# facebookresearch/DRTK

Hardware: AMD Instinct MI355X
Metric: Mpixels/sec fwd+bwd, 100k-tri @ 2048x2048, 1/2/4/8 GPU; HBM BW % (higher is better)
Workload: dtype f32; 1 GPU; 8 views/GPU x 1 GPU, 100k-tri UV-sphere head mesh (F=100352, V=50400), 2048x2048, C=16 attribute channels, transform+rasterize+render+interpolate+mask+edge_grad_estimator+loss fwd+bwd; views_per_gpu=8, triangles=100352, vertices=50400, height=2048, width=2048, channels=16, grad_reset=set_to_none, parallelism=single GPU

## Files before the change

drtk_amd/csrc/common.hpp:

```cpp
#pragma once

#include <hip/hip_runtime.h>

#include <atomic>
#include <stdint.h>
#include <string>
#include <type_traits>

#include "drtk_amd.h"

namespace drtk_amd {

constexpr int kWave = 64;
constexpr int kBlock = 256;

template <typename T>
struct Eps;
template <>
struct Eps<float> {
  static __host__ __device__ constexpr float value() { return 1e-8f; }
};
template <>
struct Eps<double> {
  static __host__ __device__ constexpr double value() { return 1e-16; }
// ... 17 lines not shown
template <typename T>
__device__ __forceinline__ T min3(T a, T b, T c) {
  T m = a;
  if (b < m) m = b;
  if (c < m) m = c;
  return m;
}
template <typename T>
__device__ __forceinline__ T max3(T a, T b, T c) {
  T m = a;
  if (m < b) m = b;
  if (m < c) m = c;
  return m;
}

__device__ __forceinline__ int lane_id() {
  return __builtin_amdgcn_mbcnt_hi(~0u, __builtin_amdgcn_mbcnt_lo(~0u, 0u));
}

template <typename T>
__device__ __forceinline__ void atomic_add_global(T* p, T v) {
  unsafeAtomicAdd(p, v);
}

template <typename T>
using NtQuad = T __attribute__((ext_vector_type(4)));
template <typename T>
__device__ __forceinline__ NtQuad<T> nt_load4(const T* p) {
  return __builtin_nontemporal_load(reinterpret_cast<const NtQuad<T>*>(p));
}
template <typename T>
__device__ __forceinline__ void nt_store4(T* p, T a, T b, T c, T d) {
  __builtin_nontemporal_store(NtQuad<T>{a, b, c, d}, reinterpret_cast<NtQuad<T>*>(p));
}

__device__ __forceinline__ int xcd_tile(int b, int n, int strip) {
  constexpr int kXcds = 8;
  const int group = kXcds * strip;
  const int base = b / group * group;
  const int r = b - base;
  const int left = n - base;
  if (left >= group) return base + (r % kXcds) * strip + r / kXcds;
  const int s = left / kXcds;
  if (r < s * kXcds) return base + (r % kXcds) * s + r / kXcds;
  return b;
}
__device__ __forceinline__ int tile_index(int strip) {
  const int b = static_cast<int>(blockIdx.x);
  return strip <= 1 ? b : xcd_tile(b, static_cast<int>(gridDim.x), strip);
}

#ifdef DRTK_AMD_ABLATION
int debug_flags();
#define DRTK_DBG(mask, bit) (((mask) & (bit)) != 0)
#else
constexpr int debug_flags() { return 0; }
#define DRTK_DBG(mask, bit) false
#endif
inline int xcd_strip(int64_t tiles_per_16_rows) {
  const int forced = (debug_flags() >> 10) & 1023;
  if (forced) return forced;
  return tiles_per_16_rows < 2 ? 2 : static_cast<int>(tiles_per_16_rows);
}

int num_compute_units();

// ... 93 lines not shown
```

drtk_amd/csrc/edge_grad.hip:

```cpp
#include <cstdlib>

#include "common.hpp"
#include "segscatter.hpp"

namespace drtk_amd {
namespace {

template <typename T>
struct Vec4;
template <>
struct Vec4<float> {
  using type = float4;
};
template <>
struct Vec4<double> {
  using type = double4;
};

template <typename T>
using Quad = T __attribute__((ext_vector_type(4), aligned(sizeof(T))));

using BufferRsrc = __amdgpu_buffer_rsrc_t;
__device__ __forceinline__ BufferRsrc buffer_rsrc(const void* base, uint32_t bytes) {
  return __builtin_amdgcn_make_buffer_rsrc(const_cast<void*>(base), 0, static_cast<int>(bytes), 0x00020000);
}
__device__ __forceinline__ float as_float(uint32_t bits) {
  return __builtin_bit_cast(float, bits);
}
__device__ __forceinline__ int32_t buffer_load_i32(BufferRsrc r, uint32_t byte_offset) {
  return static_cast<int32_t>(__builtin_amdgcn_raw_buffer_load_b32(r, byte_offset, 0, 0));
}

__device__ __forceinline__ int prefix4(int cnt, unsigned long long lt, int& total) {
  const unsigned long long b0 = __ballot(cnt & 1), b1 = __ballot(cnt & 2), b2 = __ballot(cnt & 4);
  total = __popcll(b0) + 2 * __popcll(b1) + 4 * __popcll(b2);
  return __popcll(b0 & lt) + 2 * __popcll(b1 & lt) + 4 * __popcll(b2 & lt);
}

template <typename E, typename EntryOf>
__device__ __forceinline__ void append_flagged(uint32_t f, unsigned long long lt, int& n_all, E* list, EntryOf entry) {
  int t;
  int pos = n_all + prefix4(__popc(f), lt, t);
  n_all += t;
#pragma unroll
  for (int j = 0; j < 4; ++j) {
    if (f & (1u << j)) list[pos++] = entry(j);
  }
}

template <typename T>
struct TriInfo {
  T p0x, p0y, p1x, p1y;
  T v01x, v01y, v02x, v02y, v12x, v12y;
  T den;
  T nx, ny, nz;
  int32_t i0, i1, i2;
};

template <typename T>
__device__ __forceinline__ void tri_setup(TriInfo<T>& t, T p0x, T p0y, T p1x, T p1y, T p2x, T p2y) {
  t.p0x = p0x;
  t.p0y = p0y;
  t.p1x = p1x;
  t.p1y = p1y;
// ... 1090 lines not shown
```

drtk_amd/csrc/interpolate.hip:

```cpp
#include <string>

#include "common.hpp"
#include "segscatter.hpp"

namespace drtk_amd {
namespace {

template <typename T>
struct Vec4;
template <>
struct Vec4<float> {
  using type = float4;
};
template <>
struct Vec4<double> {
  using type = double4;
};

template <typename T, int VEC, int CV, bool PREFETCH = false, bool ANYW = false>
__global__ __launch_bounds__(kBlock) void interpolate_kernel(
    const T* __restrict__ attrs, const int32_t* __restrict__ vi,
    const int32_t* __restrict__ index_img, const T* __restrict__ bary_img, int64_t V, int C,
    int64_t vi_sN, int H, int W, T* __restrict__ out, int zero_background, int strip) {
  using V4 = typename Vec4<T>::type;
// ... 416 lines not shown
      }
    }
    if (ps + 1 < kPasses) load_face(tr_next, vn);
    if constexpr (HAS_VERT) {
      int dist;
      bool tail;
      run_rows16(tr, dist, tail);
      if (__ballot(covered) != 0) {
        T p[3 * CN];
#pragma unroll
        for (int k = 0; k < 3; ++k) {
#pragma unroll
          for (int c = 0; c < CN; ++c) p[k * CN + c] = g[c] * B[k];
        }
        run_sums_rows16<T, 3 * CN>(p, dist);
        if (tail && covered) table_add<T, 3, CN, kSlots>(t_keys[wave], t_vals[wave], kStride, cur, p, attr_grad_n, CN);
      }
    }
  }
  if constexpr (HAS_VERT) {
    wave_lds_sync();
    table_flush<T, TableAcc, kSlots>(t_keys[wave], t_vals[wave], kStride, CN, attr_grad_n, CN, 0);
  }
}

constexpr int kWideWaves = 4;
constexpr int kWideWavesF64 = 3;
constexpr int kPlaneLoadAux = 2;
constexpr int kAttrGroupsAhead = 1;
constexpr bool kAnycSplitLastGroup = true;
template <typename T, bool HAS_BARY, bool TABLE, int CH, bool ANYC>
__global__ __launch_bounds__(kBlock, (sizeof(T) == 8 ? kWideWavesF64 : kWideWaves)) void interpolate_backward_wide_kernel(
    const T* __restrict__ grad_out, const T* __restrict__ attrs, const int32_t* __restrict__ vi,
    const int32_t* __restrict__ index_img, const T* __restrict__ bary_img, int64_t V, int C,
    int64_t vi_sN, int H, int W, int tiles_x, T* __restrict__ attr_grad, T* __restrict__ bary_grad,
    int dbg, int strip, int log2_slots, int CG) {
  using V4 = typename Vec4<T>::type;
  static_assert(CH % 4 == 0 && CH >= 8 && CH <= 16, "chunks of 8 or 16 channels");
  constexpr int kWaves = kBlock / kWave;
  constexpr int kPasses = kTileRows / kWaves;
  static_assert(kPasses == 4, "row pipeline below is written for 4 rows per wave");
  __shared__ __attribute__((aligned(16))) T s_g[kWaves][CH * kRunPad];
  __shared__ __attribute__((aligned(16))) T s_b[kWaves][3 * kRunPad];
  __shared__ int32_t s_vid[kWaves][3 * kRunPad];
  __shared__ int32_t s_slot[TABLE ? kWaves : 1][TABLE ? 3 * kRunPad : 1];
  extern __shared__ __attribute__((aligned(16))) unsigned char s_table_raw[];
  TableAcc* const t_vals = reinterpret_cast<TableAcc*>(s_table_raw);
  int32_t* const t_keys = reinterpret_cast<int32_t*>(t_vals + (TABLE ? (size_t(C) << log2_slots) : 0));

  const int64_t HW = int64_t(H) * W;
  const int n = blockIdx.y;
  const int tile = tile_index(strip);
  const int tyi = tile / tiles_x, txi = tile - tyi * tiles_x;
  const int wave = threadIdx.x / kWave;
  const int lane = threadIdx.x & (kWave - 1);
  const int x = txi * kWave + lane;
  const int y0 = tyi * kTileRows + wave * kPasses;
  const T* attrs_n = attrs + int64_t(n) * V * C;
  const int32_t* vi_n = vi + int64_t(n) * vi_sN;
  T* attr_grad_n = attr_grad + int64_t(n) * V * CG;
  const T* go_n = grad_out + int64_t(n) * C * HW;
  const T* bary_n = bary_img + int64_t(n) * 3 * HW;
  T* bgrad_n = HAS_BARY ? bary_grad + int64_t(n) * 3 * HW : nullptr;
  if constexpr (TABLE) {
    for (int i = threadIdx.x; i < (C << log2_slots); i += kBlock) t_vals[i] = 0;
    for (int i = threadIdx.x; i < (1 << log2_slots); i += kBlock) t_keys[i] = -1;
  }

  auto load_tr = [&](int ps) -> int32_t {
    const int y = y0 + ps;
    return (ps < kPasses && x < W && y < H) ? index_img[int64_t(n) * HW + int64_t(y) * W + x] : -1;
  };
  auto load_face = [&](int32_t t, int32_t& a0, int32_t& a1, int32_t& a2) {
    a0 = a1 = a2 = 0;
    if (t != -1) {
      const int32_t* face = vi_n + int64_t(t) * 3;
      a0 = face[0], a1 = face[1], a2 = face[2];
    }
  };

  bool wave_fg;
  {
    int32_t t4[kPasses];
#pragma unroll
    for (int ps = 0; ps < kPasses; ++ps) t4[ps] = load_tr(ps);
    const bool any_fg = (t4[0] & t4[1] & t4[2] & t4[3]) != -1;
    wave_fg = __ballot(any_fg) != 0;
    bool tile_fg = wave_fg;
    if constexpr (TABLE) tile_fg = __syncthreads_or(wave_fg) != 0;
    if (!wave_fg) {
      if constexpr (HAS_BARY) {
        int yz = y0;
        asm volatile("" : "+v"(yz));
#pragma unroll
        for (int ps = 0; ps < kPasses; ++ps) {
          const int y = yz + ps;
          if (x < W && y < H) {
            T* bgp = bgrad_n + int64_t(y) * W + x;
            bgp[0] = T(0), bgp[HW] = T(0), bgp[2 * HW] = T(0);
          }
        }
      }
      if (!TABLE || !tile_fg) return;
    }
  }

  if (wave_fg) {
  T G[CH], B[3];
  const uint32_t plane_bytes = static_cast<uint32_t>(HW * int64_t(sizeof(T)));
  auto plane_load = [&](const T* plane, uint32_t byte_offset, bool exists) -> T {
    const __amdgpu_buffer_rsrc_t r = __builtin_amdgcn_make_buffer_rsrc(const_cast<T*>(plane), 0, exists ? static_cast<int>(plane_bytes) : 0, 0x00020000);
    if constexpr (sizeof(T) == 4) {
      return __builtin_bit_cast(T, __builtin_amdgcn_raw_buffer_load_b32(r, byte_offset, 0, kPlaneLoadAux));
    } else {
      return __builtin_bit_cast(T, __builtin_amdgcn_raw_buffer_load_b64(r, byte_offset, 0, kPlaneLoadAux));
    }
  };
  auto row_offset = [&](int ps) -> uint32_t {
    return (x < W && y0 + ps < H) ? static_cast<uint32_t>((y0 + ps) * W + x) * static_cast<uint32_t>(sizeof(T)) : plane_bytes;
  };
  auto load_row = [&](int ps, int c0, int cc, bool row_any, bool with_bary) {
    if (!row_any) return;
    const uint32_t bo = row_offset(ps);
    const T* plane = go_n + int64_t(c0) * HW;
#pragma unroll
    for (int q = 0; q < CH / 4; ++q) {
      if (4 * q < cc) {
#pragma unroll
        for (int c = 4 * q; c < 4 * q + 4; ++c) {
          G[c] = plane_load(plane, bo, !ANYC || c < cc);
          plane += HW;
        }
      }
    }
    if (with_bary) {
      const T* bplane = bary_n;
#pragma unroll
      for (int k = 0; k < 3; ++k) {
        B[k] = plane_load(bplane, bo, true);
        bplane += HW;
      }
    }
  };
  int32_t tr = load_tr(0), tr_n = load_tr(1), tr_nn = -1;
  int32_t v0, v1, v2, vn0 = 0, vn1 = 0, vn2 = 0;
  load_face(tr, v0, v1, v2);
#pragma unroll
  for (int c = 0; c < CH; ++c) G[c] = T(0);
  B[0] = B[1] = B[2] = T(0);
  load_row(0, 0, min(CH, C), __ballot(tr != -1) != 0, true);
  unsigned long long heads = 0, cov = 0;
  T bg0 = T(0), bg1 = T(0), bg2 = T(0);
  int ps = 0, c0 = 0;
#pragma unroll 1
  for (;;) {
    const bool covered = tr != -1;
    if (c0 == 0) {
      if (ps + 1 < kPasses) {
        load_face(tr_n, vn0, vn1, vn2);
        tr_nn = load_tr(ps + 2);
      }
#pragma unroll
      for (int k = 0; k < 3; ++k) s_b[wave][k * kRunPad + lane] = B[k];
      s_vid[wave][0 * kRunPad + lane] = v0;
      s_vid[wave][1 * kRunPad + lane] = v1;
      s_vid[wave][2 * kRunPad + lane] = v2;
      run_masks(tr, heads, cov);
      bg0 = bg1 = bg2 = T(0);
      if constexpr (TABLE) {
        int s0 = -1, s1 = -1, s2 = -1;
        if (covered && ((heads >> lane) & 1ull) && !DRTK_DBG(dbg, 2)) {
          s0 = table_slot_rt(t_keys, v0, log2_slots);
          s1 = table_slot_rt(t_keys, v1, log2_slots);
          s2 = table_slot_rt(t_keys, v2, log2_slots);
        }
        s_slot[wave][0 * kRunPad + lane] = s0;
        s_slot[wave][1 * kRunPad + lane] = s1;
        s_slot[wave][2 * kRunPad + lane] = s2;
      }
    }
    const int cc = min(CH, C - c0);
    const bool last_chunk = c0 + CH >= C;
#pragma unroll
    for (int q = 0; q < CH / 4; ++q) {
      if (4 * q < cc) {
#pragma unroll
        for (int c = 4 * q; c < 4 * q + 4; ++c) s_g[wave][c * kRunPad + lane] = G[c];
      }
    }
    const T* a0 = attrs_n + int64_t(v0) * C + c0;
    const T* a1 = attrs_n + int64_t(v1) * C + c0;
    const T* a2 = attrs_n + int64_t(v2) * C + c0;
    constexpr int QA = kAttrGroupsAhead, QD = CH / 4 - QA;
    typedef T TQuadU __attribute__((ext_vector_type(4), aligned(sizeof(T))));
    auto attr4 = [&](const T* row, int q) -> V4 {
      if constexpr (ANYC) {
        const int ws = 4 * q + 4 <= cc ? 4 * q : cc - 4;
        const TQuadU u = *reinterpret_cast<const TQuadU*>(row + ws);
        return V4{u.x, u.y, u.z, u.w};
      } else {
        return *reinterpret_cast<const V4*>(row + 4 * q);
      }
    };
    V4 A0[QA > 0 ? QA : 1], A1[QA > 0 ? QA : 1], A2[QA > 0 ? QA : 1];
    if constexpr (HAS_BARY) {
      if (covered) {
#pragma unroll
        for (int q = 0; q < QA; ++q) {
          if (4 * q < cc) {
            A0[q] = attr4(a0, q);
            A1[q] = attr4(a1, q);
            A2[q] = attr4(a2, q);
          }
        }
      }
    }
    {
      const int n_ps = last_chunk ? ps + 1 : ps, n_c0 = last_chunk ? 0 : c0 + CH;
      const bool n_any = last_chunk ? (ps + 1 < kPasses && __ballot(tr_n != -1) != 0) : cov != 0;
      load_row(n_ps, n_c0, min(CH, C - n_c0), n_any, last_chunk);
    }
    wave_lds_sync();
    if (cov != 0 && !DRTK_DBG(dbg, 1)) {
      const T* sg = s_g[wave];
      const T* sb = s_b[wave];
      scatter_runs_rows<T, TableAcc, false, TABLE, 16, !(TABLE && HAS_BARY)>(
          heads, cov, TABLE ? s_slot[wave] : nullptr, s_vid[wave], 3 * cc, cc, t_vals, C, attr_grad_n, CG, c0, sg, sb, dbg,
          TABLE ? c0 : 0);
    }
    if constexpr (HAS_BARY) {
      if (covered && !DRTK_DBG(dbg, 8)) {
        V4 D0[QD], D1[QD], D2[QD];
        int32_t w0 = v0, w1 = v1, w2 = v2;
        asm volatile("" : "+v"(w0), "+v"(w1), "+v"(w2));
        const T* d0 = attrs_n + int64_t(w0) * C + c0;
        const T* d1 = attrs_n + int64_t(w1) * C + c0;
        const T* d2 = attrs_n + int64_t(w2) * C + c0;
        constexpr int QD1 = (ANYC && CH == 16 && kAnycSplitLastGroup && QD > 1) ? QD - 1 : QD;
#pragma unroll
        for (int q = 0; q < QD1; ++q) {
          if (4 * (QA + q) < cc) {
            D0[q] = attr4(d0, QA + q);
            D1[q] = attr4(d1, QA + q);
            D2[q] = attr4(d2, QA + q);
          }
        }
        auto dot4 = [&](int q4, const V4& u0, const V4& u1, const V4& u2) {
          if constexpr (ANYC) {
            if (4 * q4 + 4 > cc) {
// ... 17 lines not shown
          bg0 += g0 * u0.x, bg1 += g0 * u1.x, bg2 += g0 * u2.x;
          bg0 += g1 * u0.y, bg1 += g1 * u1.y, bg2 += g1 * u2.y;
          bg0 += g2 * u0.z, bg1 += g2 * u1.z, bg2 += g2 * u2.z;
          bg0 += g3 * u0.w, bg1 += g3 * u1.w, bg2 += g3 * u2.w;
        };
#pragma unroll
        for (int q = 0; q < QA; ++q) {
          if (4 * q < cc) dot4(q, A0[q], A1[q], A2[q]);
        }
#pragma unroll
        for (int q = 0; q < QD1; ++q) {
          if (4 * (QA + q) < cc) dot4(QA + q, D0[q], D1[q], D2[q]);
        }
        if constexpr (QD1 < QD) {
          if (4 * (QA + QD1) < cc) {
            asm volatile("" ::: "memory");
            const V4 e0 = attr4(d0, QA + QD1), e1 = attr4(d1, QA + QD1), e2 = attr4(d2, QA + QD1);
            dot4(QA + QD1, e0, e1, e2);
          }
        }
      }
    }
    wave_lds_sync();
    c0 += CH;
    if (last_chunk) {
      if constexpr (HAS_BARY) {
        const int y = y0 + ps;
        if (x < W && y < H) {
          T* bgp = bgrad_n + int64_t(y) * W + x;
          bgp[0] = bg0, bgp[HW] = bg1, bgp[2 * HW] = bg2;
        }
      }
      tr = tr_n, v0 = vn0, v1 = vn1, v2 = vn2;
      tr_n = tr_nn;
      c0 = 0;
      if (++ps == kPasses) break;
    }
  }
  }
  if constexpr (TABLE) {
    __syncthreads();
    if (!DRTK_DBG(dbg, 16)) {
      for (int e = threadIdx.x; e < (C << log2_slots); e += kBlock) {
        const int sl = e / C, c = e - sl * C;
        const int32_t key = t_keys[sl];
        if (key >= 0) {
          const T xv = static_cast<T>(t_vals[e]);
          if (xv != T(0)) atomic_add_global(attr_grad_n + int64_t(key) * CG + c, xv);
        }
      }
    }
  }
}

template <typename T>
__global__ __launch_bounds__(kBlock) void compact_rows_kernel(const T* __restrict__ ws, T* __restrict__ out, int64_t count, int C, int CG) {
  const int64_t i = int64_t(blockIdx.x) * kBlock + threadIdx.x;
  if (i >= count) return;
  const int64_t r = i / C;
  out[i] = ws[r * CG + (i - r * C)];
}


template <typename T>
constexpr bool kForwardPrefetch = sizeof(T) == 4;

template <typename T>
// ... 82 lines not shown
};

template <typename T>
BackwardPlan plan_backward(int64_t C, int64_t HW, bool want_attr, bool want_bary, bool cvec, bool ws_usable, bool force_generic, bool no_table) {
  BackwardPlan p;
  p.CG = static_cast<int>(C);
  const bool small_c = C <= kSmallMaxC<T> || (!want_attr && C <= kSmallInstMaxC) || (sizeof(T) == 8 && C % 4 != 0 && C <= kSmallMaxCF64Unaligned);
  if (force_generic || (!small_c && !(want_attr && HW * int64_t(sizeof(T)) < (int64_t(1) << 32)))) {
    p.route = BackwardRoute::kGeneric;
    p.cv = cvec && want_bary ? 4 : 1;
    p.generic_chunk = want_attr && C <= 4 ? 4 : 16;
  } else if (small_c) {
    p.route = BackwardRoute::kScan;
  } else {
    p.route = BackwardRoute::kWide;
    p.padded = ws_usable && !rows_are_segments<T>(C) && want_bary && sizeof(T) == 4 && C <= kPadMaxC;
    if (p.padded) p.CG = static_cast<int>(padded_row<T>(C));
    int log2_slots = 7;
    while (log2_slots > 0 && (sizeof(TableAcc) * C + 4) * (size_t(1) << log2_slots) > DRTK_INTERP_TABLE_BYTES) --log2_slots;
    p.log2_slots = log2_slots;
    p.table = log2_slots >= 4 && !p.padded && !rows_are_segments<T>(C) && !no_table;
    p.lds = p.table ? (sizeof(TableAcc) * C + 4) * (size_t(1) << p.log2_slots) : 0;
    const bool chunk12 = sizeof(T) == 4 && !cvec && C > kChunk12AboveC && C <= kChunk12MaxC && want_bary;
    p.chunk = chunk12 ? 12 : kWideChunk<T>;
  }
  return p;
}

template <typename T>
struct BackwardCall {
  const T *grad_out, *attrs;
  const int32_t *vi, *index_img;
  const T* bary_img;
  int64_t V;
  int C;
  int64_t vi_sN;
  int H, W, tiles_x;
  T *attr_grad, *bary_grad;
  int strip;
  dim3 grid;
  hipStream_t stream;
};

template <typename T, bool HAS_VERT, bool HAS_BARY, int CN>
void launch_scan(const BackwardCall<T>& c) {
  static const std::string name = instance_name<HAS_VERT, HAS_BARY, CN>("interpolate_backward_small_kernel");
  launch_as(
      name, interpolate_backward_small_kernel<T, HAS_VERT, HAS_BARY, CN>, c.grid, kBlock, 0, c.stream, c.grad_out, c.attrs, c.vi, c.index_img,
      c.bary_img, c.V, c.vi_sN, c.H, c.W, c.tiles_x, c.attr_grad, c.bary_grad, c.strip);
}
template <typename T, bool HAS_VERT, bool HAS_BARY, int CN = kSmallInstMaxC>
void launch_scan_channels(const BackwardCall<T>& c) {
  if (c.C == CN)
    launch_scan<T, HAS_VERT, HAS_BARY, CN>(c);
  else if constexpr (CN > 1)
    launch_scan_channels<T, HAS_VERT, HAS_BARY, CN - 1>(c);
}

template <typename T, bool HAS_BARY, bool TABLE, int CH, bool ANYC>
void launch_wide(const BackwardCall<T>& c, const BackwardPlan& p, T* grad_dst) {
  static const std::string name = instance_name<HAS_BARY, TABLE, CH, ANYC>("interpolate_backward_wide_kernel");
  launch_as(
      name, interpolate_backward_wide_kernel<T, HAS_BARY, TABLE, CH, ANYC>, c.grid, kBlock, p.lds, c.stream, c.grad_out, c.attrs, c.vi,
      c.index_img, c.bary_img, c.V, c.C, c.vi_sN, c.H, c.W, c.tiles_x, grad_dst, c.bary_grad, debug_flags(), c.strip, p.log2_slots, p.CG);
}
template <typename T, bool HAS_BARY, bool ANYC>
void launch_wide_chunk(const BackwardCall<T>& c, const BackwardPlan& p, T* grad_dst) {
  if constexpr (sizeof(T) == 4 && HAS_BARY && ANYC) {
    if (p.chunk == 12) return p.table ? launch_wide<T, HAS_BARY, true, 12, ANYC>(c, p, grad_dst) : launch_wide<T, HAS_BARY, false, 12, ANYC>(c, p, grad_dst);
  }
  if (p.table)
    launch_wide<T, HAS_BARY, true, kWideChunk<T>, ANYC>(c, p, grad_dst);
  else
    launch_wide<T, HAS_BARY, false, kWideChunk<T>, ANYC>(c, p, grad_dst);
}

template <typename T, bool HAS_VERT, bool HAS_BARY, int CV, int CHUNK>
void launch_generic(const BackwardCall<T>& c) {
  static const std::string name = instance_name<HAS_VERT, HAS_BARY, CV, CHUNK>("interpolate_backward_kernel");
  launch_as(
      name, interpolate_backward_kernel<T, HAS_VERT, HAS_BARY, CV, CHUNK>, c.grid, kBlock, 0, c.stream, c.grad_out, c.attrs, c.vi, c.index_img,
      c.bary_img, c.V, c.C, c.vi_sN, c.H, c.W, c.tiles_x, c.attr_grad, c.bary_grad, debug_flags(), c.strip);
}

template <typename T>
int interpolate_backward_impl(
    const T* grad_out, const T* attrs, const int32_t* vi, const int32_t* index_img,
    const T* bary_img, int64_t N, int64_t V, int64_t C, int64_t vi_sN, int64_t H, int64_t W,
    T* attr_grad, T* bary_grad, T* ws, size_t ws_bytes, hipStream_t stream) {
  const int64_t HW = H * W;
  auto zero_grad = [&](bool to_ws) -> int {
    if (!attr_grad || N * V * C == 0) return DRTK_OK;
    return to_ws ? fill_bytes_async(ws, 0, sizeof(T) * N * V * padded_row<T>(C), stream) : fill_bytes_async(attr_grad, 0, sizeof(T) * N * V * C, stream);
  };
  if (N * HW == 0 || C == 0) {
    if (zero_grad(false) != DRTK_OK) return DRTK_ERR_LAUNCH;
  }
  if (N * HW == 0) return DRTK_OK;
  if (C == 0) {
    if (bary_grad && fill_bytes_async(bary_grad, 0, sizeof(T) * N * 3 * HW, stream) != DRTK_OK) return DRTK_ERR_LAUNCH;
    return DRTK_OK;
  }
  const bool cvec = (C % 4 == 0) && (reinterpret_cast<uintptr_t>(attrs) % (4 * sizeof(T)) == 0);
  const bool ws_usable = ws && N * V * C > 0 && ws_bytes >= sizeof(T) * size_t(N * V * padded_row<T>(C)) && padded_row<T>(C) < (int64_t(1) << 30);
  const BackwardPlan p = plan_backward<T>(
      C, HW, attr_grad != nullptr, bary_grad != nullptr, cvec, ws_usable, DRTK_DBG(debug_flags(), 128), DRTK_DBG(debug_flags(), 4096));
  if (zero_grad(p.padded) != DRTK_OK) return DRTK_ERR_LAUNCH;

  const int tiles_x = static_cast<int>(ceil_div(W, kWave)), tiles_y = static_cast<int>(ceil_div(H, kTileRows));
  const BackwardCall<T> c{
      grad_out, attrs, vi, index_img, bary_img, V, (int)C, vi_sN, (int)H, (int)W, tiles_x, attr_grad, bary_grad,
      xcd_strip(int64_t(tiles_x) * (16 / kTileRows)), dim3(static_cast<unsigned>(int64_t(tiles_x) * tiles_y), static_cast<unsigned>(N)), stream};
  const bool a = attr_grad != nullptr, b = bary_grad != nullptr, v4 = p.cv == 4, c4 = p.generic_chunk == 4;
  switch (p.route) {
    case BackwardRoute::kScan:
      if (a && b) launch_scan_channels<T, true, true>(c);
      else if (a) launch_scan_channels<T, true, false>(c);
      else launch_scan_channels<T, false, true>(c);
      break;
    case BackwardRoute::kWide: {
      T* const grad_dst = p.padded ? ws : attr_grad;
      if (b && cvec) launch_wide_chunk<T, true, false>(c, p, grad_dst);
      else if (b) launch_wide_chunk<T, true, true>(c, p, grad_dst);
      else if (cvec) launch_wide_chunk<T, false, false>(c, p, grad_dst);
      else launch_wide_chunk<T, false, true>(c, p, grad_dst);
      break;
    }
    case BackwardRoute::kGeneric:
      if (a && b && c4) { if (v4) launch_generic<T, true, true, 4, 4>(c); else launch_generic<T, true, true, 1, 4>(c); }
      else if (a && b) { if (v4) launch_generic<T, true, true, 4, 16>(c); else launch_generic<T, true, true, 1, 16>(c); }
      else if (a) { if (c4) launch_generic<T, true, false, 1, 4>(c); else launch_generic<T, true, false, 1, 16>(c); }
      else { if (v4) launch_generic<T, false, true, 4, 16>(c); else launch_generic<T, false, true, 1, 16>(c); }
      break;
  }
  DRTK_RETURN_IF_LAUNCH_FAILED();
  if (p.padded) {
    const int64_t count = N * V * C;
    DRTK_LAUNCH((compact_rows_kernel<T>), dim3(static_cast<unsigned>(ceil_div(count, kBlock))), dim3(kBlock), 0, stream, ws, attr_grad, count, (int)C, p.CG);
    DRTK_RETURN_IF_LAUNCH_FAILED();
  }
  return DRTK_OK;
}

bool bad_common(int64_t N, int64_t V, int64_t C, int64_t F, int64_t vi_sN, int64_t H, int64_t W) {
// ... 45 lines not shown
}

extern "C" int drtk_amd_interpolate_backward_workspace_bytes(drtk_dtype_t dtype, int64_t N, int64_t V, int64_t C, size_t* bytes) {
  if (!bytes || N < 0 || V < 0 || C < 0) return DRTK_ERR_INVALID_ARGUMENT;
  return dispatch_dtype(dtype, [&](auto tag) {
    using T = decltype(tag);
    const BackwardPlan p = plan_backward<T>(C, 0, true, true, true, true, false, false);
    *bytes = (p.padded && N * V > 0) ? sizeof(T) * size_t(N * V * p.CG) : 0;
    return DRTK_OK;
  });
}

extern "C" int drtk_amd_interpolate_backward_ws(
    drtk_dtype_t dtype, const void* grad_out, const void* attrs, const int32_t* vi,
    const int32_t* index_img, const void* bary_img, int64_t N, int64_t V, int64_t C, int64_t F,
    int64_t vi_sN, int64_t H, int64_t W, void* attr_grad, void* bary_grad, void* workspace, size_t workspace_bytes,
    drtk_stream_t stream) {
  if (bad_common(N, V, C, F, vi_sN, H, W)) return DRTK_ERR_INVALID_ARGUMENT;
  if (!attr_grad && !bary_grad) {
    return (N * V * C > 0 && N * H * W > 0) ? DRTK_ERR_INVALID_ARGUMENT : DRTK_OK;
  }
  if (bad_inputs(dtype, attrs, vi, grad_out && index_img && bary_img, N, V, C, F, H, W)) return DRTK_ERR_INVALID_ARGUMENT;
  if (workspace && reinterpret_cast<uintptr_t>(workspace) % 64 != 0) return DRTK_ERR_INVALID_ARGUMENT;
  const size_t es = dtype_size(dtype);
  if (N > kMaxViewsPerLaunch) return for_view_slices(N, [&](int64_t n0, int64_t n) {
    return drtk_amd_interpolate_backward_ws(
        dtype, advance(grad_out, n0 * C * H * W, es), advance(attrs, n0 * V * C, es), advance_typed(vi, n0 * vi_sN),
        advance_typed(index_img, n0 * H * W), advance(bary_img, n0 * 3 * H * W, es), n, V, C, F, vi_sN, H, W,
        advance(attr_grad, n0 * V * C, es), advance(bary_grad, n0 * 3 * H * W, es), workspace, workspace_bytes, stream);
  });
  return dispatch_dtype(dtype, [&](auto tag) {
    using T = decltype(tag);
    return interpolate_backward_impl<T>(
        static_cast<const T*>(grad_out), static_cast<const T*>(attrs), vi, index_img, static_cast<const T*>(bary_img), N, V, C, vi_sN, H, W,
        static_cast<T*>(attr_grad), static_cast<T*>(bary_grad), static_cast<T*>(workspace), workspace_bytes, static_cast<hipStream_t>(stream));
  });
}

extern "C" int drtk_amd_interpolate_backward(
    drtk_dtype_t dtype, const void* grad_out, const void* attrs, const int32_t* vi,
    const int32_t* index_img, const void* bary_img, int64_t N, int64_t V, int64_t C, int64_t F,
    int64_t vi_sN, int64_t H, int64_t W, void* attr_grad, void* bary_grad, drtk_stream_t stream) {
  return drtk_amd_interpolate_backward_ws(dtype, grad_out, attrs, vi, index_img, bary_img, N, V, C, F, vi_sN, H, W, attr_grad, bary_grad, nullptr, 0, stream);
}
```

drtk_amd/csrc/render.hip:

```cpp
#include "common.hpp"
#include "segscatter.hpp"

namespace drtk_amd {
namespace {

template <typename T>
struct RenderPix {
  int32_t vi0, vi1, vi2;
  T v01x, v01y, v02x, v02y;
  T den_raw, den;
  T vp0x, vp0y;
  T b0, b1, b2;
  T z0e, z1e, z2e;
  bool z0c, z1c, z2c;
  T dinv0, dinv1, dinv2;
  T depth_inverse, depth_inverse_eps, depth;
};

template <bool EXACT, typename T>
__device__ __forceinline__ T quotient(T a, T b) {
  if constexpr (!EXACT && sizeof(T) == 4) {
    return a * __builtin_amdgcn_rcpf(b);
  } else {
    return a / b;
  }
}

template <typename T>
struct TriVerts {
  T p0x, p0y, p0z, p1x, p1y, p1z, p2x, p2y, p2z;
};

// ... 171 lines not shown
      dinv_clamped ? T(0) : quotient<false>(-dL_depth, r.depth_inverse * r.depth_inverse);

  const T dL_dinv0 = dL_B0 * r.b0 * r.depth + dL_dinv_s * r.b0;
  const T dL_dinv1 = dL_B1 * r.b1 * r.depth + dL_dinv_s * r.b1;
  const T dL_dinv2 = dL_B2 * r.b2 * r.depth + dL_dinv_s * r.b2;
  g[2] = r.z0c ? T(0) : quotient<false>(-dL_dinv0, r.z0e * r.z0e);
  g[5] = r.z1c ? T(0) : quotient<false>(-dL_dinv1, r.z1e * r.z1e);
  g[8] = r.z2c ? T(0) : quotient<false>(-dL_dinv2, r.z2e * r.z2e);

  const T dL_b0 = dL_B0 * r.dinv0 * r.depth + dL_dinv_s * r.dinv0;
  const T dL_b1 = dL_B1 * r.dinv1 * r.depth + dL_dinv_s * r.dinv1;
  const T dL_b2 = dL_B2 * r.dinv2 * r.depth + dL_dinv_s * r.dinv2;
  const T dL_b12x = -dL_b0 + dL_b1;
  const T dL_b12y = -dL_b0 + dL_b2;
  const T prex = quotient<false>(dL_b12x, r.den);
  const T prey = quotient<false>(dL_b12y, r.den);
  const T dL_den = den_clamped ? T(0) : -(prex * r.b1 + prey * r.b2);

  const T dL_vp0x = prex * r.v02y - prey * r.v01y;
  const T dL_vp0y = -prex * r.v02x + prey * r.v01x;
  const T dL_v02x = -prex * r.vp0y - dL_den * r.v01y;
  const T dL_v02y = prex * r.vp0x + dL_den * r.v01x;
  const T dL_v01x = prey * r.vp0y + dL_den * r.v02y;
  const T dL_v01y = -prey * r.vp0x - dL_den * r.v02x;

  g[0] = -dL_v02x - dL_v01x - dL_vp0x;
  g[1] = -dL_v02y - dL_v01y - dL_vp0y;
  g[3] = dL_v01x;
  g[4] = dL_v01y;
  g[6] = dL_v02x;
  g[7] = dL_v02y;
}

template <typename T>
__global__ __launch_bounds__(kBlock, sizeof(T) == 4 ? 8 : 4) void render_backward_kernel(
    const T* __restrict__ v, const int32_t* __restrict__ vi, const int32_t* __restrict__ index_img,
    const T* __restrict__ grad_depth_img, const T* __restrict__ grad_bary_img, int64_t V,
    int64_t vi_sN, int H, int W, int tiles_x, T* __restrict__ grad_v, int strip, int dbg) {
  constexpr int kWaves = kBlock / kWave;
  __shared__ int32_t t_keys[kWaves][kTableSlots];
  __shared__ TableAcc t_vals[kWaves][kTableSlots * 4];

  const int64_t HW = int64_t(H) * W;
  const int n = blockIdx.y;
  const int tile = tile_index(strip);
  const int tyi = tile / tiles_x, txi = tile - tyi * tiles_x;
  const int wave = __builtin_amdgcn_readfirstlane(threadIdx.x / kWave);
  const int lane = threadIdx.x & (kWave - 1);
  const int x = txi * kWave + lane;
  const T* v_n = v + int64_t(n) * V * 3;
  const int32_t* vi_n = vi + int64_t(n) * vi_sN;
  T* grad_v_n = grad_v + int64_t(n) * V * 3;

  table_init(t_keys[wave]);
  for (int i = lane; i < kTableSlots * 4; i += kWave) t_vals[wave][i] = 0;
  wave_lds_sync();

  auto load_tr = [&](int pass) -> int32_t {
    const int yy = tyi * kTileRows + wave * (kTileRows / kWaves) + pass;
    return (x < W && yy < H) ? index_img[int64_t(n) * HW + int64_t(yy) * W + x] : -1;
  };
  auto load_face = [&](int32_t t, int32_t (&f)[3]) {
    f[0] = f[1] = f[2] = 0;
    if (t != -1) {
      const int32_t* face = vi_n + int64_t(t) * 3;
      f[0] = face[0], f[1] = face[1], f[2] = face[2];
    }
  };
  int32_t tr_next = load_tr(0);
  int32_t vn[3];
  load_face(tr_next, vn);
#pragma unroll 1
  for (int pass = 0; pass < kTileRows / kWaves; ++pass) {
    const int y = tyi * kTileRows + wave * (kTileRows / kWaves) + pass;
    const int64_t pix = int64_t(y) * W + x;
    const int32_t tr = tr_next;
    const int32_t cur[3] = {vn[0], vn[1], vn[2]};
    if (pass + 1 < kTileRows / kWaves) tr_next = load_tr(pass + 1);
    if (__ballot(tr != -1) == 0) {
      if (pass + 1 < kTileRows / kWaves) load_face(tr_next, vn);
      continue;
    }
    T g[9];
#pragma unroll
    for (int j = 0; j < 9; ++j) g[j] = T(0);

    if (tr != -1 && DRTK_DBG(dbg, 4)) {
#pragma unroll
      for (int j = 0; j < 9; ++j) g[j] = T(1);
    } else if (tr != -1) {
      RenderPix<T> r;
      render_pix<T, false>(v_n, cur[0], cur[1], cur[2], x, y, r);
      const T* gb = grad_bary_img + int64_t(n) * 3 * HW + pix;
      render_backward_pixel<T>(r, gb[0], gb[HW], gb[2 * HW], grad_depth_img[int64_t(n) * HW + pix], g);
    }
    if (pass + 1 < kTileRows / kWaves) load_face(tr_next, vn);

    int dist;
    bool tail;
    run_rows16(tr, dist, tail);
    if (!DRTK_DBG(dbg, 1)) {
      run_sums_rows16<T, 9>(g, dist);
      if (tail && tr != -1 && !DRTK_DBG(dbg, 32)) {
        table_add<T, 3, 3>(t_keys[wave], t_vals[wave], 4, cur, g, grad_v_n, 3);
      }
    }
  }
  wave_lds_sync();
  table_flush<T>(t_keys[wave], t_vals[wave], 4, 3, grad_v_n, 3, 0);
}

template <typename T>
int render_impl(
    const T* v, const int32_t* vi, const int32_t* index_img, int64_t N, int64_t V, int64_t vi_sN,
    int64_t H, int64_t W, T* depth_img, T* bary_img, hipStream_t stream) {
  const int64_t HW = H * W;
  if (N * HW == 0) return DRTK_OK;
  const bool vec = (W % 4 == 0) && (reinterpret_cast<uintptr_t>(index_img) % 16 == 0) &&
      (reinterpret_cast<uintptr_t>(depth_img) % (4 * sizeof(T)) == 0) &&
      (reinterpret_cast<uintptr_t>(bary_img) % (4 * sizeof(T)) == 0);
  if (vec) {
    dim3 grid(static_cast<unsigned>(ceil_div(HW / 4, kBlock)), static_cast<unsigned>(N));
    DRTK_LAUNCH((render_kernel<T, 4>), grid, dim3(kBlock), 0, stream, v, vi, index_img, V, vi_sN, (int)H, (int)W, depth_img, bary_img, xcd_strip(ceil_div(16 * W, kBlock * 4)));
  } else if (W >= 4) {
    dim3 grid(static_cast<unsigned>(ceil_div(ceil_div(HW, 4), kBlock)), static_cast<unsigned>(N));
    DRTK_LAUNCH((render_kernel<T, 4, true>), grid, dim3(kBlock), 0, stream, v, vi, index_img, V, vi_sN, (int)H, (int)W, depth_img, bary_img, xcd_strip(ceil_div(16 * W, kBlock * 4)));
  } else {
    dim3 grid(static_cast<unsigned>(ceil_div(HW, kBlock)), static_cast<unsigned>(N));
    DRTK_LAUNCH((render_kernel<T, 1>), grid, dim3(kBlock), 0, stream, v, vi, index_img, V, vi_sN, (int)H, (int)W, depth_img, bary_img, xcd_strip(ceil_div(16 * W, kBlock)));
  }
  DRTK_RETURN_IF_LAUNCH_FAILED();
  return DRTK_OK;
}

template <typename T>
int render_backward_impl(
    const T* v, const int32_t* vi, const int32_t* index_img, const T* grad_depth_img,
    const T* grad_bary_img, int64_t N, int64_t V, int64_t vi_sN, int64_t H, int64_t W, T* grad_v,
    hipStream_t stream) {
  if (N * V > 0) {
    if (fill_bytes_async(grad_v, 0, sizeof(T) * N * V * 3, stream) != DRTK_OK) return DRTK_ERR_LAUNCH;
  }
  const int64_t HW = H * W;
  if (N * HW == 0) return DRTK_OK;
  const int tiles_x = static_cast<int>(ceil_div(W, kWave)), tiles_y = static_cast<int>(ceil_div(H, kTileRows));
  dim3 grid(static_cast<unsigned>(int64_t(tiles_x) * tiles_y), static_cast<unsigned>(N));
  DRTK_LAUNCH((render_backward_kernel<T>), grid, dim3(kBlock), 0, stream, v, vi, index_img, grad_depth_img, grad_bary_img, V, vi_sN, (int)H, (int)W, tiles_x, grad_v, xcd_strip(int64_t(tiles_x) * (16 / kTileRows)), debug_flags());
  DRTK_RETURN_IF_LAUNCH_FAILED();
  return DRTK_OK;
}

int check_render_args(
    bool backward, drtk_dtype_t dtype, const void* v, const int32_t* vi, const int32_t* index_img, const void* depth, const void* bary,
    int64_t N, int64_t V, int64_t F, int64_t vi_sN, int64_t H, int64_t W, const void* grad_v) {
  if (bad_image(N, H, W) || V < 0 || F < 0 || bad_view_stride(vi_sN, F * 3) || !valid_dtype(dtype)) return DRTK_ERR_INVALID_ARGUMENT;
  if (N * H * W > 0 && (!index_img || !depth || !bary)) return DRTK_ERR_INVALID_ARGUMENT;
  if ((N * V > 0 && (!v || (backward && !grad_v))) || (F > 0 && !vi)) return DRTK_ERR_INVALID_ARGUMENT;
  return DRTK_OK;
}

}
}

using namespace drtk_amd;

extern "C" int drtk_amd_render(
    drtk_dtype_t dtype, const void* v, const int32_t* vi, const int32_t* index_img, int64_t N,
    int64_t V, int64_t F, int64_t vi_sN, int64_t H, int64_t W, void* depth_img, void* bary_img,
    drtk_stream_t stream) {
  const int st = check_render_args(false, dtype, v, vi, index_img, depth_img, bary_img, N, V, F, vi_sN, H, W, nullptr);
  if (st != DRTK_OK) return st;
  const size_t es = dtype_size(dtype);
  if (N > kMaxViewsPerLaunch) return for_view_slices(N, [&](int64_t n0, int64_t n) {
    return drtk_amd_render(
        dtype, advance(v, n0 * V * 3, es), advance_typed(vi, n0 * vi_sN), advance_typed(index_img, n0 * H * W), n, V, F, vi_sN, H, W,
        advance(depth_img, n0 * H * W, es), advance(bary_img, n0 * 3 * H * W, es), stream);
  });
  return dispatch_dtype(dtype, [&](auto tag) {
    using T = decltype(tag);
    return render_impl<T>(
        static_cast<const T*>(v), vi, index_img, N, V, vi_sN, H, W, static_cast<T*>(depth_img), static_cast<T*>(bary_img),
        static_cast<hipStream_t>(stream));
  });
}

extern "C" int drtk_amd_render_backward(
    drtk_dtype_t dtype, const void* v, const int32_t* vi, const int32_t* index_img,
    const void* grad_depth_img, const void* grad_bary_img, int64_t N, int64_t V, int64_t F,
    int64_t vi_sN, int64_t H, int64_t W, void* grad_v, drtk_stream_t stream) {
  const int st = check_render_args(true, dtype, v, vi, index_img, grad_depth_img, grad_bary_img, N, V, F, vi_sN, H, W, grad_v);
  if (st != DRTK_OK) return st;
  const size_t es = dtype_size(dtype);
  if (N > kMaxViewsPerLaunch) return for_view_slices(N, [&](int64_t n0, int64_t n) {
    return drtk_amd_render_backward(
        dtype, advance(v, n0 * V * 3, es), advance_typed(vi, n0 * vi_sN), advance_typed(index_img, n0 * H * W),
        advance(grad_depth_img, n0 * H * W, es), advance(grad_bary_img, n0 * 3 * H * W, es), n, V, F, vi_sN, H, W,
        advance(grad_v, n0 * V * 3, es), stream);
  });
  return dispatch_dtype(dtype, [&](auto tag) {
    using T = decltype(tag);
    return render_backward_impl<T>(
        static_cast<const T*>(v), vi, index_img, static_cast<const T*>(grad_depth_img), static_cast<const T*>(grad_bary_img), N, V,
        vi_sN, H, W, static_cast<T*>(grad_v), static_cast<hipStream_t>(stream));
  });
}
```

Before: 7382 Mpix/s.

## Use buffer-descriptor loads and batched prefetch in render and interpolate backward

Adds a float-only render_backward path that builds buffer resource descriptors for the index, face, vertex and gradient planes. It issues all four rows' index and face loads up front, using out-of-range offsets instead of branches so masked lanes read zero, and pins the results with empty asm to keep loads batched. The interpolate backward wide kernel gets the same treatment: its four index rows load at once through a descriptor and the next-face prefetch moves later in the loop. The aim is to expose more memory-level parallelism and drop branchy guarded loads, at the cost of more live registers and a 32-bit offset limit on sizes.

```diff
diff --git a/drtk_amd/csrc/common.hpp b/drtk_amd/csrc/common.hpp
--- a/drtk_amd/csrc/common.hpp
+++ b/drtk_amd/csrc/common.hpp
@@ -73,6 +73,20 @@
 template <typename T>
 __device__ __forceinline__ void nt_store4(T* p, T a, T b, T c, T d) {
   __builtin_nontemporal_store(NtQuad<T>{a, b, c, d}, reinterpret_cast<NtQuad<T>*>(p));
+}
+
+using BufferRsrc = __amdgpu_buffer_rsrc_t;
+__device__ __forceinline__ BufferRsrc buffer_rsrc(const void* base, uint32_t bytes) {
+  return __builtin_amdgcn_make_buffer_rsrc(const_cast<void*>(base), 0, static_cast<int>(bytes), 0x00020000);
+}
+__device__ __forceinline__ float as_float(uint32_t bits) {
+  return __builtin_bit_cast(float, bits);
+}
+__device__ __forceinline__ int32_t buffer_load_i32(BufferRsrc r, uint32_t byte_offset) {
+  return static_cast<int32_t>(__builtin_amdgcn_raw_buffer_load_b32(r, byte_offset, 0, 0));
+}
+__device__ __forceinline__ float buffer_load_f32(BufferRsrc r, uint32_t byte_offset) {
+  return as_float(__builtin_amdgcn_raw_buffer_load_b32(r, byte_offset, 0, 0));
 }
 
 __device__ __forceinline__ int xcd_tile(int b, int n, int strip) {
diff --git a/drtk_amd/csrc/edge_grad.hip b/drtk_amd/csrc/edge_grad.hip
--- a/drtk_amd/csrc/edge_grad.hip
+++ b/drtk_amd/csrc/edge_grad.hip
@@ -20,16 +20,6 @@
 template <typename T>
 using Quad = T __attribute__((ext_vector_type(4), aligned(sizeof(T))));
 
-using BufferRsrc = __amdgpu_buffer_rsrc_t;
-__device__ __forceinline__ BufferRsrc buffer_rsrc(const void* base, uint32_t bytes) {
-  return __builtin_amdgcn_make_buffer_rsrc(const_cast<void*>(base), 0, static_cast<int>(bytes), 0x00020000);
-}
-__device__ __forceinline__ float as_float(uint32_t bits) {
-  return __builtin_bit_cast(float, bits);
-}
-__device__ __forceinline__ int32_t buffer_load_i32(BufferRsrc r, uint32_t byte_offset) {
-  return static_cast<int32_t>(__builtin_amdgcn_raw_buffer_load_b32(r, byte_offset, 0, 0));
-}
 
 __device__ __forceinline__ int prefix4(int cnt, unsigned long long lt, int& total) {
   const unsigned long long b0 = __ballot(cnt & 1), b1 = __ballot(cnt & 2), b2 = __ballot(cnt & 4);
diff --git a/drtk_amd/csrc/interpolate.hip b/drtk_amd/csrc/interpolate.hip
--- a/drtk_amd/csrc/interpolate.hip
+++ b/drtk_amd/csrc/interpolate.hip
@@ -472,7 +472,7 @@
 template <typename T, bool HAS_BARY, bool TABLE, int CH, bool ANYC>
 __global__ __launch_bounds__(kBlock, (sizeof(T) == 8 ? kWideWavesF64 : kWideWaves)) void interpolate_backward_wide_kernel(
     const T* __restrict__ grad_out, const T* __restrict__ attrs, const int32_t* __restrict__ vi,
-    const int32_t* __restrict__ index_img, const T* __restrict__ bary_img, int64_t V, int C,
+    const int32_t* __restrict__ index_img, const T* __restrict__ bary_img, int64_t V, int64_t F, int C,
     int64_t vi_sN, int H, int W, int tiles_x, T* __restrict__ attr_grad, T* __restrict__ bary_grad,
     int dbg, int strip, int log2_slots, int CG) {
   using V4 = typename Vec4<T>::type;
@@ -507,23 +507,25 @@
     for (int i = threadIdx.x; i < (1 << log2_slots); i += kBlock) t_keys[i] = -1;
   }
 
-  auto load_tr = [&](int ps) -> int32_t {
-    const int y = y0 + ps;
-    return (ps < kPasses && x < W && y < H) ? index_img[int64_t(n) * HW + int64_t(y) * W + x] : -1;
+  const uint32_t idx_bytes = static_cast<uint32_t>(HW) * 4u, vi_bytes = static_cast<uint32_t>(F) * 12u;
+  const BufferRsrc idx_rsrc = buffer_rsrc(index_img + int64_t(n) * HW, idx_bytes);
+  const BufferRsrc vi_rsrc = buffer_rsrc(vi_n, vi_bytes);
+  auto load_face = [&](int32_t t, int32_t& a0, int32_t& a1, int32_t& a2) {
+    const auto f = __builtin_amdgcn_raw_buffer_load_b96(vi_rsrc, t != -1 ? static_cast<uint32_t>(t) * 12u : vi_bytes, 0, 0);
+    a0 = static_cast<int32_t>(f[0]), a1 = static_cast<int32_t>(f[1]), a2 = static_cast<int32_t>(f[2]);
   };
-  auto load_face = [&](int32_t t, int32_t& a0, int32_t& a1, int32_t& a2) {
-    a0 = a1 = a2 = 0;
-    if (t != -1) {
-      const int32_t* face = vi_n + int64_t(t) * 3;
-      a0 = face[0], a1 = face[1], a2 = face[2];
-    }
-  };
 
   bool wave_fg;
+  int32_t t4[kPasses];
   {
-    int32_t t4[kPasses];
-#pragma unroll
-    for (int ps = 0; ps < kPasses; ++ps) t4[ps] = load_tr(ps);
+#pragma unroll
+    for (int ps = 0; ps < kPasses; ++ps) {
+      const uint32_t o = (static_cast<uint32_t>(y0 + ps) * static_cast<uint32_t>(W) + static_cast<uint32_t>(x)) * 4u;
+      t4[ps] = buffer_load_i32(idx_rsrc, (x < W && y0 + ps < H) ? o : idx_bytes);
+    }
+    asm volatile("" : "+v"(t4[0]), "+v"(t4[1]), "+v"(t4[2]), "+v"(t4[3]));
+#pragma unroll
+    for (int ps = 0; ps < kPasses; ++ps) t4[ps] = (x < W && y0 + ps < H) ? t4[ps] : -1;
     const bool any_fg = (t4[0] & t4[1] & t4[2] & t4[3]) != -1;
     wave_fg = __ballot(any_fg) != 0;
     bool tile_fg = wave_fg;
@@ -582,13 +584,14 @@
       }
     }
   };
-  int32_t tr = load_tr(0), tr_n = load_tr(1), tr_nn = -1;
+  int32_t tr = t4[0], tr_n = t4[1], tr_nn = t4[2], tr_nnn = t4[3];
   int32_t v0, v1, v2, vn0 = 0, vn1 = 0, vn2 = 0;
   load_face(tr, v0, v1, v2);
 #pragma unroll
   for (int c = 0; c < CH; ++c) G[c] = T(0);
   B[0] = B[1] = B[2] = T(0);
   load_row(0, 0, min(CH, C), __ballot(tr != -1) != 0, true);
+  asm volatile("" : "+v"(v0), "+v"(v1), "+v"(v2));
   unsigned long long heads = 0, cov = 0;
   T bg0 = T(0), bg1 = T(0), bg2 = T(0);
   int ps = 0, c0 = 0;
@@ -596,10 +599,6 @@
   for (;;) {
     const bool covered = tr != -1;
     if (c0 == 0) {
-      if (ps + 1 < kPasses) {
-        load_face(tr_n, vn0, vn1, vn2);
-        tr_nn = load_tr(ps + 2);
-      }
 #pragma unroll
       for (int k = 0; k < 3; ++k) s_b[wave][k * kRunPad + lane] = B[k];
       s_vid[wave][0 * kRunPad + lane] = v0;
@@ -655,6 +654,7 @@
         }
       }
     }
+    if (c0 == 0) load_face(tr_n, vn0, vn1, vn2);
     {
       const int n_ps = last_chunk ? ps + 1 : ps, n_c0 = last_chunk ? 0 : c0 + CH;
       const bool n_any = last_chunk ? (ps + 1 < kPasses && __ballot(tr_n != -1) != 0) : cov != 0;
@@ -738,7 +738,7 @@
         }
       }
       tr = tr_n, v0 = vn0, v1 = vn1, v2 = vn2;
-      tr_n = tr_nn;
+      tr_n = tr_nn, tr_nn = tr_nnn, tr_nnn = -1;
       c0 = 0;
       if (++ps == kPasses) break;
     }
@@ -887,7 +887,7 @@
   const T *grad_out, *attrs;
   const int32_t *vi, *index_img;
   const T* bary_img;
-  int64_t V;
+  int64_t V, F;
   int C;
   int64_t vi_sN;
   int H, W, tiles_x;
@@ -917,7 +917,7 @@
   static const std::string name = instance_name<HAS_BARY, TABLE, CH, ANYC>("interpolate_backward_wide_kernel");
   launch_as(
       name, interpolate_backward_wide_kernel<T, HAS_BARY, TABLE, CH, ANYC>, c.grid, kBlock, p.lds, c.stream, c.grad_out, c.attrs, c.vi,
-      c.index_img, c.bary_img, c.V, c.C, c.vi_sN, c.H, c.W, c.tiles_x, grad_dst, c.bary_grad, debug_flags(), c.strip, p.log2_slots, p.CG);
+      c.index_img, c.bary_img, c.V, c.F, c.C, c.vi_sN, c.H, c.W, c.tiles_x, grad_dst, c.bary_grad, debug_flags(), c.strip, p.log2_slots, p.CG);
 }
 template <typename T, bool HAS_BARY, bool ANYC>
 void launch_wide_chunk(const BackwardCall<T>& c, const BackwardPlan& p, T* grad_dst) {
@@ -941,7 +941,7 @@
 template <typename T>
 int interpolate_backward_impl(
     const T* grad_out, const T* attrs, const int32_t* vi, const int32_t* index_img,
-    const T* bary_img, int64_t N, int64_t V, int64_t C, int64_t vi_sN, int64_t H, int64_t W,
+    const T* bary_img, int64_t N, int64_t V, int64_t C, int64_t F, int64_t vi_sN, int64_t H, int64_t W,
     T* attr_grad, T* bary_grad, T* ws, size_t ws_bytes, hipStream_t stream) {
   const int64_t HW = H * W;
   auto zero_grad = [&](bool to_ws) -> int {
@@ -958,13 +958,14 @@
   }
   const bool cvec = (C % 4 == 0) && (reinterpret_cast<uintptr_t>(attrs) % (4 * sizeof(T)) == 0);
   const bool ws_usable = ws && N * V * C > 0 && ws_bytes >= sizeof(T) * size_t(N * V * padded_row<T>(C)) && padded_row<T>(C) < (int64_t(1) << 30);
+  const int64_t HW_plan = F < (int64_t(1) << 32) / 12 ? HW : (int64_t(1) << 32);
   const BackwardPlan p = plan_backward<T>(
-      C, HW, attr_grad != nullptr, bary_grad != nullptr, cvec, ws_usable, DRTK_DBG(debug_flags(), 128), DRTK_DBG(debug_flags(), 4096));
+      C, HW_plan, attr_grad != nullptr, bary_grad != nullptr, cvec, ws_usable, DRTK_DBG(debug_flags(), 128), DRTK_DBG(debug_flags(), 4096));
   if (zero_grad(p.padded) != DRTK_OK) return DRTK_ERR_LAUNCH;
 
   const int tiles_x = static_cast<int>(ceil_div(W, kWave)), tiles_y = static_cast<int>(ceil_div(H, kTileRows));
   const BackwardCall<T> c{
-      grad_out, attrs, vi, index_img, bary_img, V, (int)C, vi_sN, (int)H, (int)W, tiles_x, attr_grad, bary_grad,
+      grad_out, attrs, vi, index_img, bary_img, V, F, (int)C, vi_sN, (int)H, (int)W, tiles_x, attr_grad, bary_grad,
       xcd_strip(int64_t(tiles_x) * (16 / kTileRows)), dim3(static_cast<unsigned>(int64_t(tiles_x) * tiles_y), static_cast<unsigned>(N)), stream};
   const bool a = attr_grad != nullptr, b = bary_grad != nullptr, v4 = p.cv == 4, c4 = p.generic_chunk == 4;
   switch (p.route) {
@@ -1076,7 +1077,7 @@
   return dispatch_dtype(dtype, [&](auto tag) {
     using T = decltype(tag);
     return interpolate_backward_impl<T>(
-        static_cast<const T*>(grad_out), static_cast<const T*>(attrs), vi, index_img, static_cast<const T*>(bary_img), N, V, C, vi_sN, H, W,
+        static_cast<const T*>(grad_out), static_cast<const T*>(attrs), vi, index_img, static_cast<const T*>(bary_img), N, V, C, F, vi_sN, H, W,
         static_cast<T*>(attr_grad), static_cast<T*>(bary_grad), static_cast<T*>(workspace), workspace_bytes, static_cast<hipStream_t>(stream));
   });
 }
diff --git a/drtk_amd/csrc/render.hip b/drtk_amd/csrc/render.hip
--- a/drtk_amd/csrc/render.hip
+++ b/drtk_amd/csrc/render.hip
@@ -1,3 +1,5 @@
+#include <cstdlib>
+
 #include "common.hpp"
 #include "segscatter.hpp"
 
@@ -235,10 +237,16 @@
   g[7] = dL_v02y;
 }
 
-template <typename T>
+
+struct RenderBwdRow {
+  TriVerts<float> q;
+  float gd, gb0, gb1, gb2;
+};
+
+template <typename T, bool BUF>
 __global__ __launch_bounds__(kBlock, sizeof(T) == 4 ? 8 : 4) void render_backward_kernel(
     const T* __restrict__ v, const int32_t* __restrict__ vi, const int32_t* __restrict__ index_img,
-    const T* __restrict__ grad_depth_img, const T* __restrict__ grad_bary_img, int64_t V,
+    const T* __restrict__ grad_depth_img, const T* __restrict__ grad_bary_img, int64_t V, int64_t F,
     int64_t vi_sN, int H, int W, int tiles_x, T* __restrict__ grad_v, int strip, int dbg) {
   constexpr int kWaves = kBlock / kWave;
   __shared__ int32_t t_keys[kWaves][kTableSlots];
@@ -259,6 +267,84 @@
   for (int i = lane; i < kTableSlots * 4; i += kWave) t_vals[wave][i] = 0;
   wave_lds_sync();
 
+  if constexpr (BUF) {
+    static_assert(sizeof(T) == 4, "the descriptor body is written for float");
+    constexpr int kRows = kTileRows / kWaves;
+    const uint32_t plane_bytes = static_cast<uint32_t>(HW) * 4u;
+    const uint32_t vi_bytes = static_cast<uint32_t>(F) * 12u, v_bytes = static_cast<uint32_t>(V) * 12u;
+    const T* gb_n = grad_bary_img + int64_t(n) * 3 * HW;
+    const BufferRsrc idx_rsrc = buffer_rsrc(index_img + int64_t(n) * HW, plane_bytes);
+    const BufferRsrc vi_rsrc = buffer_rsrc(vi_n, vi_bytes);
+    const BufferRsrc v_rsrc = buffer_rsrc(v_n, v_bytes);
+    const BufferRsrc gd_rsrc = buffer_rsrc(grad_depth_img + int64_t(n) * HW, plane_bytes);
+    const BufferRsrc gb0_rsrc = buffer_rsrc(gb_n, plane_bytes);
+    const BufferRsrc gb1_rsrc = buffer_rsrc(gb_n + HW, plane_bytes);
+    const BufferRsrc gb2_rsrc = buffer_rsrc(gb_n + 2 * HW, plane_bytes);
+    const int y0 = tyi * kTileRows + wave * kRows;
+    int32_t tr[kRows], f[kRows][3];
+    auto row_off = [&](int p) -> uint32_t {
+      const uint32_t o = (static_cast<uint32_t>(y0 + p) * static_cast<uint32_t>(W) + static_cast<uint32_t>(x)) * 4u;
+      return (x < W && y0 + p < H) ? o : plane_bytes;
+    };
+#pragma unroll
+    for (int p = 0; p < kRows; ++p) tr[p] = buffer_load_i32(idx_rsrc, row_off(p));
+    asm volatile("" : "+v"(tr[0]), "+v"(tr[1]), "+v"(tr[2]), "+v"(tr[3]));
+#pragma unroll
+    for (int p = 0; p < kRows; ++p) tr[p] = (x < W && y0 + p < H) ? tr[p] : -1;
+    if (__ballot((tr[0] & tr[1] & tr[2] & tr[3]) != -1) != 0) {
+#pragma unroll
+    for (int p = 0; p < kRows; ++p) {
+      const auto c = __builtin_amdgcn_raw_buffer_load_b96(vi_rsrc, tr[p] != -1 ? static_cast<uint32_t>(tr[p]) * 12u : vi_bytes, 0, 0);
+#pragma unroll
+      for (int k = 0; k < 3; ++k) f[p][k] = static_cast<int32_t>(c[k]);
+    }
+    asm volatile("" : "+v"(f[0][0]), "+v"(f[0][1]), "+v"(f[0][2]), "+v"(f[1][0]), "+v"(f[1][1]), "+v"(f[1][2]),
+                      "+v"(f[2][0]), "+v"(f[2][1]), "+v"(f[2][2]), "+v"(f[3][0]), "+v"(f[3][1]), "+v"(f[3][2]));
+    auto pin_row = [](RenderBwdRow& r) {
+      asm volatile("" : "+v"(r.q.p0x), "+v"(r.q.p0y), "+v"(r.q.p0z), "+v"(r.q.p1x), "+v"(r.q.p1y), "+v"(r.q.p1z), "+v"(r.q.p2x),
+                        "+v"(r.q.p2y), "+v"(r.q.p2z), "+v"(r.gd), "+v"(r.gb0), "+v"(r.gb1), "+v"(r.gb2));
+    };
+    auto load_row = [&](int p) -> RenderBwdRow {
+      const bool covered = tr[p] != -1;
+      const uint32_t goff = covered ? row_off(p) : plane_bytes;
+      const auto a = __builtin_amdgcn_raw_buffer_load_b96(v_rsrc, covered ? static_cast<uint32_t>(f[p][0]) * 12u : v_bytes, 0, 0);
+      const auto b = __builtin_amdgcn_raw_buffer_load_b96(v_rsrc, covered ? static_cast<uint32_t>(f[p][1]) * 12u : v_bytes, 0, 0);
+      const auto c = __builtin_amdgcn_raw_buffer_load_b96(v_rsrc, covered ? static_cast<uint32_t>(f[p][2]) * 12u : v_bytes, 0, 0);
+      RenderBwdRow r;
+      r.gd = buffer_load_f32(gd_rsrc, goff);
+      r.gb0 = buffer_load_f32(gb0_rsrc, goff);
+      r.gb1 = buffer_load_f32(gb1_rsrc, goff);
+      r.gb2 = buffer_load_f32(gb2_rsrc, goff);
+      r.q = TriVerts<float>{as_float(a[0]), as_float(a[1]), as_float(a[2]), as_float(b[0]), as_float(b[1]), as_float(b[2]),
+                            as_float(c[0]), as_float(c[1]), as_float(c[2])};
+      return r;
+    };
+#pragma unroll
+    for (int p = 0; p < kRows; ++p) {
+      const bool covered = tr[p] != -1;
+      const bool row_any = __ballot(covered) != 0;
+      RenderBwdRow in = load_row(p);
+      pin_row(in);
+      if (row_any) {
+        T g[9];
+        RenderPix<T> r;
+        render_math<T, false>(in.q, f[p][0], f[p][1], f[p][2], x, y0 + p, r);
+        render_backward_pixel<T>(r, in.gb0, in.gb1, in.gb2, in.gd, g);
+#pragma unroll
+        for (int j = 0; j < 9; ++j) g[j] = covered ? (DRTK_DBG(dbg, 4) ? T(1) : g[j]) : T(0);
+        int dist;
+        bool tail;
+        run_rows16(tr[p], dist, tail);
+        if (!DRTK_DBG(dbg, 1)) {
+          run_sums_rows16<T, 9>(g, dist);
+          if (tail && covered && !DRTK_DBG(dbg, 32)) {
+            table_add<T, 3, 3>(t_keys[wave], t_vals[wave], 4, f[p], g, grad_v_n, 3);
+          }
+        }
+      }
+    }
+    }
+  } else {
   auto load_tr = [&](int pass) -> int32_t {
     const int yy = tyi * kTileRows + wave * (kTileRows / kWaves) + pass;
     return (x < W && yy < H) ? index_img[int64_t(n) * HW + int64_t(yy) * W + x] : -1;
@@ -308,6 +394,7 @@
         table_add<T, 3, 3>(t_keys[wave], t_vals[wave], 4, cur, g, grad_v_n, 3);
       }
     }
+  }
   }
   wave_lds_sync();
   table_flush<T>(t_keys[wave], t_vals[wave], 4, 3, grad_v_n, 3, 0);
@@ -337,9 +424,17 @@
 }
 
 template <typename T>
+bool render_backward_buffer_body(int64_t HW, int64_t V, int64_t F) {
+  if (sizeof(T) != 4) return false;
+  const char* e = std::getenv("DRTK_AMD_RENDER_BACKWARD_BUFFER");
+  if (e && e[0] == '0' && !e[1]) return false;
+  return HW < (int64_t(1) << 30) && V < (int64_t(1) << 32) / 12 && F < (int64_t(1) << 32) / 12;
+}
+
+template <typename T>
 int render_backward_impl(
     const T* v, const int32_t* vi, const int32_t* index_img, const T* grad_depth_img,
-    const T* grad_bary_img, int64_t N, int64_t V, int64_t vi_sN, int64_t H, int64_t W, T* grad_v,
+    const T* grad_bary_img, int64_t N, int64_t V, int64_t F, int64_t vi_sN, int64_t H, int64_t W, T* grad_v,
     hipStream_t stream) {
   if (N * V > 0) {
     if (fill_bytes_async(grad_v, 0, sizeof(T) * N * V * 3, stream) != DRTK_OK) return DRTK_ERR_LAUNCH;
@@ -348,7 +443,15 @@
   if (N * HW == 0) return DRTK_OK;
   const int tiles_x = static_cast<int>(ceil_div(W, kWave)), tiles_y = static_cast<int>(ceil_div(H, kTileRows));
   dim3 grid(static_cast<unsigned>(int64_t(tiles_x) * tiles_y), static_cast<unsigned>(N));
-  DRTK_LAUNCH((render_backward_kernel<T>), grid, dim3(kBlock), 0, stream, v, vi, index_img, grad_depth_img, grad_bary_img, V, vi_sN, (int)H, (int)W, tiles_x, grad_v, xcd_strip(int64_t(tiles_x) * (16 / kTileRows)), debug_flags());
+  const int strip = xcd_strip(int64_t(tiles_x) * (16 / kTileRows));
+  if constexpr (sizeof(T) == 4) {
+    if (render_backward_buffer_body<T>(HW, V, F)) {
+      DRTK_LAUNCH((render_backward_kernel<T, true>), grid, dim3(kBlock), 0, stream, v, vi, index_img, grad_depth_img, grad_bary_img, V, F, vi_sN, (int)H, (int)W, tiles_x, grad_v, strip, debug_flags());
+      DRTK_RETURN_IF_LAUNCH_FAILED();
+      return DRTK_OK;
+    }
+  }
+  DRTK_LAUNCH((render_backward_kernel<T, false>), grid, dim3(kBlock), 0, stream, v, vi, index_img, grad_depth_img, grad_bary_img, V, F, vi_sN, (int)H, (int)W, tiles_x, grad_v, strip, debug_flags());
   DRTK_RETURN_IF_LAUNCH_FAILED();
   return DRTK_OK;
 }
@@ -404,6 +507,6 @@
     using T = decltype(tag);
     return render_backward_impl<T>(
         static_cast<const T*>(v), vi, index_img, static_cast<const T*>(grad_depth_img), static_cast<const T*>(grad_bary_img), N, V,
-        vi_sN, H, W, static_cast<T*>(grad_v), static_cast<hipStream_t>(stream));
+        F, vi_sN, H, W, static_cast<T*>(grad_v), static_cast<hipStream_t>(stream));
   });
 }
```

Result: no change. 7429 Mpix/s (median of 6 runs) (+0.6%).
